# genglongling/EE274_ConvexCaldera_LLM_quantization

Hardware: AMD Instinct MI355X
Metric: weight matrices/sec (4096x4096, rank-128, Q=2-bit) + Frob err vs ref (higher is better)
Workload: dtype f32 (fp16 W in; fp32-grade split-fp16 MFMA products, fp64 small solves; int2 codes)

## Files before the change

ee274_convexcaldera_llm_quantization_amd/csrc/cq_small.hip:

```cpp
#include "cq_common.h"

namespace cq {

constexpr int GT = 64;
constexpr int GK = 32;
constexpr int kGramThreads = 256;

__global__ __launch_bounds__(kGramThreads) void gram_f64_kernel(
    int64_t M, int64_t N, int64_t K, int64_t kchunk, int splits, const float* __restrict__ A,
    int ta, int64_t lda, int64_t sa, const float* __restrict__ B, int tb, int64_t ldb, int64_t sb,
    double* __restrict__ part, const int* __restrict__ active) {
    __shared__ float As[GK][GT + 1];
    __shared__ float Bs[GK][GT + 1];
    const int64_t b = blockIdx.z / splits;
    if (active && !active[b]) return;
    const int split = blockIdx.z % splits;
    const int64_t i0 = (int64_t)blockIdx.y * GT, j0 = (int64_t)blockIdx.x * GT;
    const float* Ab = A + b * sa;
    const float* Bb = B + b * sb;
    const int tx = threadIdx.x & 15, ty = threadIdx.x >> 4;
    double acc[4][4];
#pragma unroll
    for (int u = 0; u < 4; ++u)
#pragma unroll
        for (int v = 0; v < 4; ++v) acc[u][v] = 0.0;
    const int64_t kbeg = split * kchunk, kend = min(K, kbeg + kchunk);
    for (int64_t k0 = kbeg; k0 < kend; k0 += GK) {
        for (int e = threadIdx.x; e < GK * GT; e += kGramThreads) {
            int kk, ii;
            if (!ta) { kk = e / GT; ii = e % GT; } else { ii = e / GK; kk = e % GK; }
            const int64_t gk = k0 + kk, gi = i0 + ii;
            float v = 0.f;
            if (gk < kend && gi < M) v = ta ? Ab[gi * lda + gk] : Ab[gk * lda + gi];
            As[kk][ii] = v;
            int jj;
            if (!tb) { kk = e / GT; jj = e % GT; } else { jj = e / GK; kk = e % GK; }
            const int64_t gk2 = k0 + kk, gj = j0 + jj;
            float w = 0.f;
            if (gk2 < kend && gj < N) w = tb ? Bb[gj * ldb + gk2] : Bb[gk2 * ldb + gj];
            Bs[kk][jj] = w;
        }
        __syncthreads();
#pragma unroll 4
        for (int kk = 0; kk < GK; ++kk) {
            double av[4], bv[4];
#pragma unroll
            for (int u = 0; u < 4; ++u) av[u] = (double)As[kk][ty * 4 + u];
#pragma unroll
            for (int v = 0; v < 4; ++v) bv[v] = (double)Bs[kk][tx * 4 + v];
#pragma unroll
            for (int u = 0; u < 4; ++u)
#pragma unroll
                for (int v = 0; v < 4; ++v) acc[u][v] = fma(av[u], bv[v], acc[u][v]);
        }
        __syncthreads();
    }
    double* P = part + ((int64_t)b * splits + split) * M * N;
#pragma unroll
    for (int u = 0; u < 4; ++u)
#pragma unroll
        for (int v = 0; v < 4; ++v) {
            const int64_t i = i0 + ty * 4 + u, j = j0 + tx * 4 + v;
            if (i < M && j < N) P[i * N + j] = acc[u][v];
        }
}

__global__ void gram_reduce_kernel(const double* __restrict__ part, int64_t MN, int splits,
                                   int64_t batch, double* __restrict__ C, const int* __restrict__ active) {
    const int64_t total = batch * MN;
    for (int64_t e = (int64_t)blockIdx.x * blockDim.x + threadIdx.x; e < total;
         e += (int64_t)gridDim.x * blockDim.x) {
        const int64_t b = e / MN, o = e % MN;
        if (active && !active[b]) continue;
        double s = 0.0;
        for (int t = 0; t < splits; ++t) s += part[(b * splits + t) * MN + o];
        C[e] = s;
    }
}


using f64x4v = __attribute__((ext_vector_type(4))) double;

template <bool TK>
__global__ __launch_bounds__(kGramThreads) void gram_f64_mfma_kernel(
    int64_t M, int64_t N, int64_t K, int64_t kchunk, int splits, const float* __restrict__ A,
    int64_t lda, int64_t sa, const float* __restrict__ B, int64_t ldb, int64_t sb, int sym,
    double* __restrict__ part, double* __restrict__ C, const int* __restrict__ active) {
    constexpr int GP = TK ? GT + 4 : GT + 16;
    __shared__ float As[2][GK][GP];
    __shared__ float Bs[2][GK][GP];
    const int64_t b = blockIdx.z / splits;
    const int split = blockIdx.z % splits;
    if (sym && blockIdx.x < blockIdx.y) return;
    if (active && !active[b]) return;
    const int64_t i0 = (int64_t)blockIdx.y * GT, j0 = (int64_t)blockIdx.x * GT;
    const float* Ab = A + b * sa;
    const float* Bb = B + b * sb;
    const int t = threadIdx.x, lane = t & 63, wid = t >> 6;
    const int wi = wid >> 1, wj = wid & 1;
    const int lr = t >> 4, lc = (t & 15) * 4;
    const int tr = t >> 3, tk = (t & 7) * 4;
    const int64_t kbeg = split * kchunk, kend = min(K, kbeg + kchunk);
    auto ld4 = [&](const float* base, int64_t ld, int64_t lim, int64_t k, int64_t c0) -> float4 {
        float4 v = make_float4(0.f, 0.f, 0.f, 0.f);
        if (k < kend) {
            const float* src = base + k * ld + c0;
            if (c0 + 3 < lim) v = *reinterpret_cast<const float4*>(src);
            else {
                if (c0 < lim) v.x = src[0];
                if (c0 + 1 < lim) v.y = src[1];
                if (c0 + 2 < lim) v.z = src[2];
            }
        }
        return v;
    };
    f64x4v acc[2][2];
#pragma unroll
    for (int u = 0; u < 2; ++u)
#pragma unroll
        for (int v = 0; v < 2; ++v) acc[u][v] = f64x4v{0.0, 0.0, 0.0, 0.0};
    float4 ra[2], rb[2];
    auto ld4t = [&](const float* base, int64_t ld, int64_t lim, int64_t row, int64_t k) -> float4 {
        float4 v = make_float4(0.f, 0.f, 0.f, 0.f);
        if (row < lim && k < kend) {
            const float* src = base + row * ld + k;
            if (k + 3 < kend) v = *reinterpret_cast<const float4*>(src);
            else {
                v.x = src[0];
                if (k + 1 < kend) v.y = src[1];
                if (k + 2 < kend) v.z = src[2];
            }
        }
        return v;
    };
    auto fetch = [&](int64_t k0) {
#pragma unroll
        for (int h = 0; h < 2; ++h) {
            if constexpr (TK) {
                ra[h] = ld4t(Ab, lda, M, i0 + tr + 32 * h, k0 + tk);
                rb[h] = ld4t(Bb, ldb, N, j0 + tr + 32 * h, k0 + tk);
            } else {
                ra[h] = ld4(Ab, lda, M, k0 + lr + 16 * h, i0 + lc);
                rb[h] = ld4(Bb, ldb, N, k0 + lr + 16 * h, j0 + lc);
            }
        }
    };
    auto stash = [&](int buf) {
#pragma unroll
        for (int h = 0; h < 2; ++h) {
            if constexpr (TK) {
                const int c = tr + 32 * h;
                As[buf][tk + 0][c] = ra[h].x; As[buf][tk + 1][c] = ra[h].y;
                As[buf][tk + 2][c] = ra[h].z; As[buf][tk + 3][c] = ra[h].w;
                Bs[buf][tk + 0][c] = rb[h].x; Bs[buf][tk + 1][c] = rb[h].y;
                Bs[buf][tk + 2][c] = rb[h].z; Bs[buf][tk + 3][c] = rb[h].w;
            } else {
                *reinterpret_cast<float4*>(&As[buf][lr + 16 * h][lc]) = ra[h];
                *reinterpret_cast<float4*>(&Bs[buf][lr + 16 * h][lc]) = rb[h];
            }
        }
    };
    const int nsl = (int)ceil_div(kend - kbeg, GK);
    if (nsl > 0) { fetch(kbeg); stash(0); }
    __syncthreads();
    const int li = lane & 15, lk = lane >> 4;
    for (int sl = 0; sl < nsl; ++sl) {
        const int cur = sl & 1;
        if (sl + 1 < nsl) fetch(kbeg + (int64_t)(sl + 1) * GK);
#pragma unroll
        for (int kk = 0; kk < GK; kk += 4) {
            double a0 = (double)As[cur][kk + lk][32 * wi + li];
            double a1 = (double)As[cur][kk + lk][32 * wi + 16 + li];
            double b0 = (double)Bs[cur][kk + lk][32 * wj + li];
            double b1 = (double)Bs[cur][kk + lk][32 * wj + 16 + li];
            acc[0][0] = __builtin_amdgcn_mfma_f64_16x16x4f64(a0, b0, acc[0][0], 0, 0, 0);
            acc[0][1] = __builtin_amdgcn_mfma_f64_16x16x4f64(a0, b1, acc[0][1], 0, 0, 0);
            acc[1][0] = __builtin_amdgcn_mfma_f64_16x16x4f64(a1, b0, acc[1][0], 0, 0, 0);
            acc[1][1] = __builtin_amdgcn_mfma_f64_16x16x4f64(a1, b1, acc[1][1], 0, 0, 0);
        }
        if (sl + 1 < nsl) stash(1 - cur);
        __syncthreads();
    }
    double* P = C ? C + (int64_t)b * M * N : part + ((int64_t)b * splits + split) * M * N;
    const bool mirror = C && sym && blockIdx.x != blockIdx.y;
#pragma unroll
    for (int u = 0; u < 2; ++u)
#pragma unroll
        for (int v = 0; v < 2; ++v)
#pragma unroll
            for (int r = 0; r < 4; ++r) {
                const int64_t i = i0 + 32 * wi + 16 * u + lk + 4 * r;
                const int64_t j = j0 + 32 * wj + 16 * v + li;
                if (i < M && j < N) {
                    const double x = C ? 0.0 + acc[u][v][r] : acc[u][v][r];
                    P[i * N + j] = x;
                    if (mirror) P[j * N + i] = x;
                }
            }
}

__global__ void gram_reduce_sym_kernel(const double* __restrict__ part, int64_t M, int splits,
                                       int64_t batch, double* __restrict__ C, const int* __restrict__ active) {
    const int64_t MN = M * M, total = batch * MN;
    for (int64_t e = (int64_t)blockIdx.x * blockDim.x + threadIdx.x; e < total;
         e += (int64_t)gridDim.x * blockDim.x) {
        const int64_t b = e / MN, o = e % MN, i = o / M, j = o % M;
        if (active && !active[b]) continue;
        const int64_t src = (i / GT > j / GT) ? j * M + i : o;
        double s = 0.0;
        for (int t2 = 0; t2 < splits; ++t2) s += part[(b * splits + t2) * MN + src];
        C[e] = s;
    }
}

static int gram_splits(int64_t M, int64_t N, int64_t K, int64_t batch) {
    const int64_t tiles = ceil_div(M, GT) * ceil_div(N, GT) * batch;
    int64_t s = ceil_div(1024, tiles);
    s = std::min<int64_t>(s, std::max<int64_t>(1, K / 256));
    return (int)std::max<int64_t>(1, std::min<int64_t>(s, 64));
}

template <int PPT, int RPT, int JBR, int NTH>
__global__ __launch_bounds__(NTH) void jacobi_reg_kernel(const double* __restrict__ A_all,
                                                                    int p, int max_sweeps, double tol,
                                                                    double* __restrict__ evals,
                                                                    float* __restrict__ V32,
                                                                    double* __restrict__ V64,
                                                                    int* __restrict__ sweeps_out,
                                                                    const int* __restrict__ active) {
    extern __shared__ __attribute__((aligned(16))) char smem_raw[];
    if (active && !active[blockIdx.x]) {
        if (threadIdx.x == 0 && sweeps_out) sweeps_out[blockIdx.x] = 0;
        return;
    }
    const int P = p + (p & 1);
    const int H = P / 2;
    double2* csn = reinterpret_cast<double2*>(smem_raw);
    int4* lohi = reinterpret_cast<int4*>(csn + H);
    int* flp = reinterpret_cast<int*>(lohi + H);
    int* seat = flp + H;
    int* seat2 = seat + P;
    int* rnk = seat2 + P;
    double* a = reinterpret_cast<double*>(rnk + P + ((9 * H + 3 * P) & 1));
    __shared__ double red[16];
    __shared__ int stop;
    const int64_t b = blockIdx.x;
    const double* Ag = A_all + b * (int64_t)p * p;
    const int tid = threadIdx.x, lane = tid & 63, wid = tid >> 6;
    const bool wantv = V32 != nullptr || V64 != nullptr;
    const int pg = lane & 31;
    const int rg = 2 * wid + (lane >> 5);
    const int k0 = pg * PPT, x0 = rg * RPT;
    auto pk = [p](int i, int j) -> int {
        if (i > j) { const int t = i; i = j; j = t; }
        return i * p - ((i * (i - 1)) >> 1) + (j - i);
    };
    auto pko = [p](int i) -> int { return i * p - ((i * (i - 1)) >> 1) - i; };
    auto pkx = [](int x, int ox, int y, int oy) -> int { return x <= y ? ox + y : oy + x; };
    for (int i = wid; i < p; i += (NTH / 64))
        for (int c = lane; c < p; c += 64)
            if (c >= i) a[pk(i, c)] = 0.5 * (Ag[i * p + c] + Ag[c * p + i]);
    for (int s = tid; s < P; s += NTH) seat[s] = s;
    float ev[PPT][RPT], od[PPT][RPT];
#pragma unroll
    for (int u = 0; u < PPT; ++u)
#pragma unroll
        for (int r = 0; r < RPT; ++r) {
            const int k = k0 + u, x = x0 + r;
            ev[u][r] = (x == 2 * k) ? 1.f : 0.f;
            od[u][r] = (x == 2 * k + 1) ? 1.f : 0.f;
        }
    __syncthreads();
    const double skip_rel = fmax(1e-17, 0.01 * tol);
    const double skip_rel2 = skip_rel * skip_rel;
    constexpr int JMB = 5;
    const int nblk = H * (H + 1) / 2;
    int bqa[JMB], bqb[JMB];
#pragma unroll
    for (int u = 0; u < JMB; ++u) {
        const int e = tid + u * NTH;
        bqa[u] = -1;
        bqb[u] = 0;
        if (JBR == 1 && e < nblk) {
            int qb = (int)((sqrtf(8.0f * (float)e + 1.0f) - 1.0f) * 0.5f);
            if (qb * (qb + 1) / 2 > e) --qb;
            if ((qb + 1) * (qb + 2) / 2 <= e) ++qb;
            bqa[u] = e - qb * (qb + 1) / 2;
            bqb[u] = qb;
        }
    }
    int* scur = seat;
    int* snxt = seat2;
    int sweep = 0;
    for (; sweep < max_sweeps; ++sweep) {
        double off = 0.0, dg = 0.0;
        for (int i = wid; i < p; i += (NTH / 64))
            for (int c = i + lane; c < p; c += 64) {
                const double v = a[pk(i, c)];
                if (c == i) dg += v * v; else off += 2.0 * v * v;
            }
        const double offs = block_sum_f64(off, red);
        const double dgs = block_sum_f64(dg, red);
        if (tid == 0) stop = (offs <= tol * tol * dgs) ? 1 : 0;
        __syncthreads();
        if (stop) break;
        for (int rd = 0; rd < P - 1; ++rd) {
            int act = 0;
            for (int k = tid; k < H; k += NTH) {
                const int se = scur[2 * k], so = scur[2 * k + 1];
                const int i = min(se, so), j = max(se, so);
                double c = 1.0, s = 0.0;
                if (j < p) {
                    const double aij = a[pk(i, j)];
                    const double aii = a[pk(i, i)], ajj = a[pk(j, j)];
                    if (fabs(aij) > 1e-300 && aij * aij > skip_rel2 * fabs(aii * ajj)) {
                        const double th = (ajj - aii) / (2.0 * aij);
                        const double t = (th >= 0 ? 1.0 : -1.0) / (fabs(th) + sqrt(1.0 + th * th));
                        c = 1.0 / sqrt(1.0 + t * t);
                        s = t * c;
                        act = 1;
                    }
                }
                csn[k] = make_double2(c, s); lohi[k] = make_int4(i, j, pko(i), pko(j)); flp[k] = se > so;
                snxt[2 * k] = (k == 0) ? se : (k == 1) ? scur[1] : scur[2 * k - 2];
                snxt[2 * k + 1] = (k == H - 1) ? se : scur[2 * k + 3];
            }
            const bool any = __syncthreads_or(act);
            if (any) {
                if constexpr (JBR == 1) {
#pragma unroll
                    for (int u = 0; u < JMB; ++u) {
                        const int qa = bqa[u], qb = bqb[u];
                        if (qa < 0) continue;
                        const double2 rca = csn[qa], rcb = csn[qb];
                        const double sa = rca.y, sb = rcb.y;
                        if (sa == 0.0 && sb == 0.0) continue;
                        const double ca = rca.x, cb = rcb.x;
                        const int4 pa = lohi[qa], pb = lohi[qb];
                        const int ia = pa.x, ja = pa.y, ib = pb.x, jb = pb.y;
                        const int oia = pa.z, oja = pa.w, oib = pb.z, ojb = pb.w;
                        const bool va = ja < p, vb = jb < p;
                        if (qa == qb) {
                            if (!va) continue;
                            const int o0 = pkx(ia, oia, ia, oia), o1 = pkx(ia, oia, ja, oja), o3 = pkx(ja, oja, ja, oja);
                            const double x0 = a[o0], x1 = a[o1], x3 = a[o3];
                            const double y00 = cb * x0 - sb * x1, y01 = sb * x0 + cb * x1;
                            const double y10 = cb * x1 - sb * x3, y11 = sb * x1 + cb * x3;
                            a[o0] = ca * y00 - sa * y10;
                            a[o3] = sa * y01 + ca * y11;
                            a[o1] = 0.0;
                        } else {
                            const int o0 = pkx(ia, oia, ib, oib);
                            const int o1 = vb ? pkx(ia, oia, jb, ojb) : -1;
                            const int o2 = va ? pkx(ja, oja, ib, oib) : -1;
                            const int o3 = (va && vb) ? pkx(ja, oja, jb, ojb) : -1;
                            const double x0 = a[o0];
                            const double x1 = o1 >= 0 ? a[o1] : 0.0;
                            const double x2 = o2 >= 0 ? a[o2] : 0.0;
                            const double x3 = o3 >= 0 ? a[o3] : 0.0;
                            const double y00 = cb * x0 - sb * x1, y01 = sb * x0 + cb * x1;
                            const double y10 = cb * x2 - sb * x3, y11 = sb * x2 + cb * x3;
                            a[o0] = ca * y00 - sa * y10;
                            if (o1 >= 0) a[o1] = ca * y01 - sa * y11;
                            if (o2 >= 0) a[o2] = sa * y00 + ca * y10;
                            if (o3 >= 0) a[o3] = sa * y01 + ca * y11;
                        }
                    }
                } else
                for (int e0 = tid; e0 < nblk; e0 += NTH * JBR) {
                    int o[JBR][4];
                    double x[JBR][4], ca[JBR], sa[JBR], cb[JBR], sb[JBR];
                    bool live[JBR], dgn[JBR];
#pragma unroll
                    for (int u = 0; u < JBR; ++u) {
                        const int e = e0 + u * NTH;
                        live[u] = false;
                        dgn[u] = false;
                        if (e < nblk) {
                            int qb = (int)((sqrtf(8.0f * (float)e + 1.0f) - 1.0f) * 0.5f);
                            if (qb * (qb + 1) / 2 > e) --qb;
                            if ((qb + 1) * (qb + 2) / 2 <= e) ++qb;
                            const int qa = e - qb * (qb + 1) / 2;
                            ca[u] = csn[qa].x; sa[u] = csn[qa].y; cb[u] = csn[qb].x; sb[u] = csn[qb].y;
                            const int ia = lohi[qa].x, ja = lohi[qa].y, ib = lohi[qb].x, jb = lohi[qb].y;
                            const bool va = ja < p, vb = jb < p;
                            if ((sa[u] != 0.0 || sb[u] != 0.0) && (qa != qb || va)) {
                                live[u] = true;
                                dgn[u] = (qa == qb);
                                if (dgn[u]) {
                                    o[u][0] = pk(ia, ia); o[u][1] = pk(ia, ja);
                                    o[u][2] = o[u][1]; o[u][3] = pk(ja, ja);
                                } else {
                                    o[u][0] = pk(ia, ib);
                                    o[u][1] = vb ? pk(ia, jb) : -1;
                                    o[u][2] = va ? pk(ja, ib) : -1;
                                    o[u][3] = (va && vb) ? pk(ja, jb) : -1;
                                }
#pragma unroll
                                for (int w4 = 0; w4 < 4; ++w4) x[u][w4] = o[u][w4] >= 0 ? a[o[u][w4]] : 0.0;
                            }
                        }
                    }
#pragma unroll
                    for (int u = 0; u < JBR; ++u) {
                        if (!live[u]) continue;
                        const double y00 = cb[u] * x[u][0] - sb[u] * x[u][1], y01 = sb[u] * x[u][0] + cb[u] * x[u][1];
                        const double y10 = cb[u] * x[u][2] - sb[u] * x[u][3], y11 = sb[u] * x[u][2] + cb[u] * x[u][3];
                        if (dgn[u]) {
                            a[o[u][0]] = ca[u] * y00 - sa[u] * y10;
                            a[o[u][3]] = sa[u] * y01 + ca[u] * y11;
                            a[o[u][1]] = 0.0;
                        } else {
                            a[o[u][0]] = ca[u] * y00 - sa[u] * y10;
                            if (o[u][1] >= 0) a[o[u][1]] = ca[u] * y01 - sa[u] * y11;
                            if (o[u][2] >= 0) a[o[u][2]] = sa[u] * y00 + ca[u] * y10;
                            if (o[u][3] >= 0) a[o[u][3]] = sa[u] * y01 + ca[u] * y11;
                        }
                    }
                }
#pragma unroll
                for (int u = 0; u < PPT; ++u) {
                    if (!wantv) break;
                    const int k = k0 + u;
                    if (k < H) {
                        const float c = (float)csn[k].x, s = (float)csn[k].y;
                        if (s != 0.f) {
                            const bool f = flp[k] != 0;
#pragma unroll
                            for (int r = 0; r < RPT; ++r) {
                                const float e = ev[u][r], o2 = od[u][r];
                                if (!f) { ev[u][r] = c * e - s * o2; od[u][r] = s * e + c * o2; }
                                else { od[u][r] = c * o2 - s * e; ev[u][r] = s * o2 + c * e; }
                            }
                        }
                    }
                }
            }
#pragma unroll
            for (int r = 0; r < RPT; ++r) {
                if (!wantv) break;
                const float from_left = __shfl_up(ev[PPT - 1][r], 1, 32);
                const float from_right = __shfl_down(od[0][r], 1, 32);
                float ne[PPT], no[PPT];
#pragma unroll
                for (int u = 0; u < PPT; ++u) {
                    const int k = k0 + u;
                    const float evm1 = (u == 0) ? from_left : ev[u - 1][r];
                    const float odp1 = (u == PPT - 1) ? from_right : od[u + 1][r];
                    ne[u] = (k == 0) ? ev[u][r] : (k == 1) ? od[u - (u > 0 ? 1 : 0)][r] : evm1;
                    no[u] = (k == H - 1) ? ev[u][r] : odp1;
                    if (k >= H) { ne[u] = ev[u][r]; no[u] = od[u][r]; }
                }
                const float od0_left = __shfl_up(od[PPT - 1][r], 1, 32);
                if (PPT == 1 && k0 == 1) ne[0] = od0_left;
#pragma unroll
                for (int u = 0; u < PPT; ++u) { ev[u][r] = ne[u]; od[u][r] = no[u]; }
            }
            __syncthreads();
            int* const t2 = scur;
            scur = snxt;
            snxt = t2;
        }
    }
    if (tid == 0 && sweeps_out) sweeps_out[b] = sweep;
    for (int i = tid; i < p; i += NTH) {
        const double di = a[pk(i, i)];
        int rank = 0;
        for (int j = 0; j < p; ++j) {
            const double dj = a[pk(j, j)];
            rank += (dj > di) || (dj == di && j < i);
        }
        evals[b * p + rank] = di;
        rnk[i] = rank;
    }
    __syncthreads();
#pragma unroll
    for (int u = 0; u < PPT; ++u) {
        const int k = k0 + u;
        if (k >= H) continue;
        const int pe = scur[2 * k], po = scur[2 * k + 1];
#pragma unroll
        for (int r = 0; r < RPT; ++r) {
            const int x = x0 + r;
            if (x >= p) continue;
            if (pe < p) {
                if (V32) V32[b * (int64_t)p * p + x * p + rnk[pe]] = ev[u][r];
                if (V64) V64[b * (int64_t)p * p + x * p + rnk[pe]] = ev[u][r];
            }
            if (po < p) {
                if (V32) V32[b * (int64_t)p * p + x * p + rnk[po]] = od[u][r];
                if (V64) V64[b * (int64_t)p * p + x * p + rnk[po]] = od[u][r];
            }
        }
    }
}

static size_t jacobi_reg_bytes(int p) {
    const int P = p + (p & 1), H = P / 2;
    return (size_t)2 * H * sizeof(double) + (size_t)(5 * H + 3 * P + 1) * sizeof(int) + 8 +
           (size_t)p * (p + 1) / 2 * sizeof(double) + 16;
}

constexpr int kWmThreads = 512;
__host__ __device__ inline int wm_pitch(int p) { return p + (48 - p % 32) % 32; }
constexpr int kWmWaves = kWmThreads / 64;


template <bool LP>
__global__ __launch_bounds__(kWmThreads) void spd_whiten_mfma_kernel(double* __restrict__ S_all, int p, double rc2,
                                                                     double* __restrict__ E_all,
                                                                     float* __restrict__ W32, int* __restrict__ info,
                                                                     const int* __restrict__ active) {
    extern __shared__ __attribute__((aligned(16))) double wm_smem[];
    if (active && !active[blockIdx.x]) return;
    double* piv = wm_smem;
    double* Li = piv + p;
    double* rp = Li + 32 * 33;
    double* Bk = rp + 32;
    const int pp = wm_pitch(p);
    double* PP = Bk + 32 * 33;
    __shared__ int bad;
    __shared__ double dmax_s;
    __shared__ double red[16];
    const int64_t b = blockIdx.x;
    double* S = S_all + b * (int64_t)p * p;
    double* E = E_all + b * (int64_t)p * p;
    const int tid = threadIdx.x, lane = tid & 63, wid = tid >> 6;
    const int l16 = lane & 15, lk = lane >> 4;
    for (int i = wid; i < p; i += kWmWaves)
        for (int c = lane; c < p; c += 64) E[(int64_t)i * p + c] = (i == c) ? 1.0 : 0.0;
    double dm = 0.0;
    for (int j = tid; j < p; j += kWmThreads) dm = fmax(dm, fabs(S[(int64_t)j * p + j]));
    for (int o = 32; o > 0; o >>= 1) {
        const int2 x = __builtin_bit_cast(int2, dm);
        int2 y;
        y.x = __shfl_xor(x.x, o, 64);
        y.y = __shfl_xor(x.y, o, 64);
        dm = fmax(dm, __builtin_bit_cast(double, y));
    }
    if (lane == 0) red[wid] = dm;
    if (tid == 0) bad = 0;
    __syncthreads();
    if (tid == 0) {
        double m = 0.0;
        for (int w = 0; w < kWmWaves; ++w) m = fmax(m, red[w]);
        dmax_s = m;
    }
    __syncthreads();
    const double dmax = dmax_s;
    for (int J = 0; J < p; J += 32) {
        const int nb = min(32, p - J);
        const int t0 = J + nb;
        {
            const int r = tid >> 4, c0 = tid & 15;
#pragma unroll
            for (int h = 0; h < 2; ++h) {
                const int c = c0 + 16 * h;
                const int a = min(r, c), e = max(r, c);
                Bk[r * 33 + c] = (r < nb && c < nb) ? S[(int64_t)(J + a) * p + J + e] : 0.0;
                Li[r * 33 + c] = (c == r) ? 1.0 : 0.0;
            }
            __syncthreads();
            int nbad = 0;
            for (int k = 0; k < nb; ++k) {
                const double d = Bk[k * 33 + k];
                const bool drop = !(d > 1e-300 && d > dmax * rc2);
                nbad += drop;
                if (tid == 0) {
                    piv[J + k] = drop ? __longlong_as_double(0x7ff0000000000000ll) : d;
                    rp[k] = drop ? 0.0 : 1.0 / d;
                }
                if (!drop && r > k && r < nb) {
                    const double f = Bk[r * 33 + k] / d;
#pragma unroll
                    for (int h = 0; h < 2; ++h) {
                        const int c = c0 + 16 * h;
                        if (c > k && c < nb) Bk[r * 33 + c] -= f * Bk[k * 33 + c];
                        else if (c <= k) Li[r * 33 + c] -= f * Li[k * 33 + c];
                    }
                }
                __syncthreads();
            }
            if (tid == 0) bad += nbad;
        }
        __syncthreads();
        const int ncs = (p - t0 + 15) / 16, nce = (t0 + 15) / 16;
        for (int cb = wid; cb < ncs + nce; cb += kWmWaves) {
            const bool isS = cb < ncs;
            double* M = isS ? S : E;
            const int c0 = isS ? t0 + 16 * cb : 16 * (cb - ncs);
            const int clim = isS ? p : t0;
            const int col = c0 + l16;
            f64x4v acc[2] = {f64x4v{0.0, 0.0, 0.0, 0.0}, f64x4v{0.0, 0.0, 0.0, 0.0}};
#pragma unroll
            for (int k0 = 0; k0 < 32; k0 += 4) {
                const int k = k0 + lk;
                const double bv = (k < nb && col < clim) ? M[(int64_t)(J + k) * p + col] : 0.0;
                acc[0] = __builtin_amdgcn_mfma_f64_16x16x4f64(Li[l16 * 33 + k], bv, acc[0], 0, 0, 0);
                acc[1] = __builtin_amdgcn_mfma_f64_16x16x4f64(Li[(16 + l16) * 33 + k], bv, acc[1], 0, 0, 0);
            }
#pragma unroll
            for (int h = 0; h < 2; ++h)
#pragma unroll
                for (int r = 0; r < 4; ++r) {
                    const int k = 16 * h + lk + 4 * r;
                    if (col < clim) {
                        const double v = k < nb ? acc[h][r] : 0.0;
                        if (LP) PP[k * pp + col] = v;
                        if ((!isS || !LP) && k < nb) M[(int64_t)(J + k) * p + col] = v;
                    }
                }
        }
        __syncthreads();
        const int nt = (p - t0 + 15) / 16;
        const int nst = nt * (nt + 1) / 2, net = nt * nce;
        auto tile_of = [&](int t, int& i0, int& c0, double*& M) {
            if (t < nst) {
                int tj = (int)((sqrtf(8.0f * (float)t + 1.0f) - 1.0f) * 0.5f);
                if (tj * (tj + 1) / 2 > t) --tj;
                if ((tj + 1) * (tj + 2) / 2 <= t) ++tj;
                i0 = t0 + 16 * (t - tj * (tj + 1) / 2);
                c0 = t0 + 16 * tj;
                M = S;
            } else {
                i0 = t0 + 16 * ((t - nst) / nce);
                c0 = 16 * ((t - nst) % nce);
                M = E;
            }
        };
        for (int t = wid; t < nst + net; t += 2 * kWmWaves) {
            const int tb = t + kWmWaves;
            const bool two = tb < nst + net;
            int i0[2] = {0, 0}, c0[2] = {0, 0};
            double* M[2] = {S, S};
            tile_of(t, i0[0], c0[0], M[0]);
            if (two) tile_of(tb, i0[1], c0[1], M[1]);
            double dv[2][4];
#pragma unroll
            for (int u = 0; u < 2; ++u) {
                const int clim = (M[u] == S) ? p : t0;
                const int col = c0[u] + l16;
#pragma unroll
                for (int r = 0; r < 4; ++r) {
                    const int i = i0[u] + lk + 4 * r;
                    dv[u][r] = (u == 0 || two) && i < p && col < clim ? M[u][(int64_t)i * p + col] : 0.0;
                }
            }
#pragma unroll
            for (int u = 0; u < 2; ++u) {
                if (u == 1 && !two) break;
                const int clim = (M[u] == S) ? p : t0;
                const int col = c0[u] + l16, arow = i0[u] + l16;
                f64x4v acc = f64x4v{0.0, 0.0, 0.0, 0.0};
#pragma unroll
                for (int k0 = 0; k0 < 32; k0 += 4) {
                    const int k = k0 + lk;
                    const bool kv = k < nb;
                    const double av = (kv && arow < p) ? (LP ? PP[k * pp + arow] : S[(int64_t)(J + k) * p + arow]) * rp[k] : 0.0;
                    const double bv = (kv && col < clim) ? (LP ? PP[k * pp + col] : M[u][(int64_t)(J + k) * p + col]) : 0.0;
                    acc = __builtin_amdgcn_mfma_f64_16x16x4f64(av, bv, acc, 0, 0, 0);
                }
#pragma unroll
                for (int r = 0; r < 4; ++r) {
                    const int i = i0[u] + lk + 4 * r;
                    if (i < p && col < clim) M[u][(int64_t)i * p + col] = dv[u][r] - acc[r];
                }
            }
        }
        __syncthreads();
    }
    if (tid == 0) info[b] = bad;
    for (int a = wid; a < p; a += kWmWaves)
        for (int c = lane; c < p; c += 64) {
            const double v = (c >= a) ? E[(int64_t)c * p + a] / sqrt(piv[c]) : 0.0;
            if (W32) W32[b * (int64_t)p * p + (int64_t)a * p + c] = (float)v;
            S[(int64_t)a * p + c] = v;
        }
}

constexpr int kLzThreads = 256, kLzMaxP = 192, kLzMaxPG = 512, kLzMaxSteps = 64;

__device__ __forceinline__ int lz_sturm(const double* al, const double* b2, int m, double x) {
    int cnt = 0;
    double d = 1.0;
    for (int k = 0; k < m; ++k) {
        d = (al[k] - x) - (k > 0 ? b2[k] / d : 0.0);
        if (d == 0.0) d = -1e-300;
        cnt += d < 0.0;
    }
    return cnt;
}

template <int Q, bool GT, int NT>
__global__ __launch_bounds__(NT) void extreme_eigs_kernel(const double* __restrict__ T_all, int p, int steps,
                                                         double* __restrict__ ends,
                                                         const int* __restrict__ active) {
    if (active && !active[blockIdx.x]) return;
    extern __shared__ __attribute__((aligned(16))) float lz_t[];
    __shared__ float vf[64 * Q];
    __shared__ float part[NT / 64][64 * Q];
    __shared__ double al[kLzMaxSteps], b2[kLzMaxSteps];
    __shared__ int m_s;
    const int64_t b = blockIdx.x;
    const double* T = T_all + b * (int64_t)p * p;
    const int tid = threadIdx.x, lane = tid & 63, wid = tid >> 6;
    if constexpr (!GT) {
        for (int e = tid; e < p * p; e += NT) lz_t[e] = (float)T[e];
        __syncthreads();
        for (int e = tid; e < p * p; e += NT) {
            const int j = e / p, i = e % p;
            if (i < j) {
                const float v = 0.5f * (lz_t[e] + lz_t[i * p + j]);
                lz_t[e] = v;
                lz_t[i * p + j] = v;
            }
        }
    }
    double v[Q], vp[Q];
#pragma unroll
    for (int q = 0; q < Q; ++q) v[q] = vp[q] = 0.0;
    if (wid == 0) {
        double ss = 0.0;
#pragma unroll
        for (int q = 0; q < Q; ++q) {
            const int i = lane + 64 * q;
            if (i < p) {
                uint32_t h = (uint32_t)i * 2654435761u ^ 0x9E3779B9u;
                h ^= h >> 16; h *= 0x7feb352du; h ^= h >> 15;
                v[q] = ((double)(h & 0xffffu) / 65536.0 + 0.5) * ((h & 0x10000u) ? 1.0 : -1.0);
                ss += v[q] * v[q];
            }
        }
        const double inv = 1.0 / sqrt(wave_sum(ss));
#pragma unroll
        for (int q = 0; q < Q; ++q) {
            v[q] *= inv;
            if (lane + 64 * q < p) vf[lane + 64 * q] = (float)v[q];
        }
        if (lane == 0) m_s = steps;
    }
    __syncthreads();
    constexpr int NWV = NT / 64;
    const int jc = (p + NWV - 1) / NWV, j0 = wid * jc, j1 = min(p, j0 + jc);
    double beta = 0.0;
    for (int k = 0; k < steps; ++k) {
        {
            int ii[Q];
            float a[Q];
#pragma unroll
            for (int q = 0; q < Q; ++q) {
                ii[q] = lane + 64 * q < p ? lane + 64 * q : 0;
                a[q] = 0.f;
            }
            int j = j0;
            for (; j + 4 <= j1; j += 4) {
                float t[4][Q], vj[4];
#pragma unroll
                for (int u = 0; u < 4; ++u) {
                    vj[u] = vf[j + u];
#pragma unroll
                    for (int q = 0; q < Q; ++q)
                        t[u][q] = GT ? (float)T[(int64_t)(j + u) * p + ii[q]] : lz_t[(j + u) * p + ii[q]];
                }
#pragma unroll
                for (int u = 0; u < 4; ++u)
#pragma unroll
                    for (int q = 0; q < Q; ++q) a[q] = __builtin_fmaf(t[u][q], vj[u], a[q]);
            }
            for (; j < j1; ++j) {
                const float vj = vf[j];
#pragma unroll
                for (int q = 0; q < Q; ++q)
                    a[q] = __builtin_fmaf(GT ? (float)T[(int64_t)j * p + ii[q]] : lz_t[j * p + ii[q]], vj, a[q]);
            }
#pragma unroll
            for (int q = 0; q < Q; ++q)
                if (lane + 64 * q < p) part[wid][lane + 64 * q] = a[q];
        }
        __syncthreads();
        if (wid == 0) {
            double w[Q], a = 0.0;
#pragma unroll
            for (int q = 0; q < Q; ++q) {
                const int i = lane + 64 * q;
                w[q] = 0.0;
                if (i < p) {
                    double acc = 0.0;
#pragma unroll
                    for (int wv = 0; wv < NWV; ++wv) acc += (double)part[wv][i];
                    w[q] = acc;
                    w[q] -= beta * vp[q];
                    a += w[q] * v[q];
                }
            }
            a = wave_sum(a);
            double ss = 0.0;
#pragma unroll
            for (int q = 0; q < Q; ++q) {
                w[q] -= a * v[q];
                ss += w[q] * w[q];
            }
            ss = wave_sum(ss);
            if (lane == 0) {
                al[k] = a;
                b2[k + 1 < kLzMaxSteps ? k + 1 : 0] = ss;
            }
            beta = sqrt(ss);
            const int stop = !(beta > 1e-30 * fabs(a)) || k + 1 == steps;
            if (stop && lane == 0) m_s = k + 1;
            const double inv = stop ? 0.0 : 1.0 / beta;
#pragma unroll
            for (int q = 0; q < Q; ++q) {
                vp[q] = v[q];
                v[q] = w[q] * inv;
                if (lane + 64 * q < p) vf[lane + 64 * q] = (float)v[q];
            }
        }
        __syncthreads();
        if (m_s != steps || k + 1 == steps) break;
    }
    const int m = m_s;
    if (wid < 2) {
        double lo = INFINITY, hi = -INFINITY;
        for (int k = 0; k < m; ++k) {
            const double r = (k > 0 ? sqrt(b2[k]) : 0.0) + (k + 1 < m ? sqrt(b2[k + 1]) : 0.0);
            lo = fmin(lo, al[k] - r);
            hi = fmax(hi, al[k] + r);
        }
        const double pad = 1e-12 * fmax(fabs(lo), fabs(hi)) + 1e-300;
        double a = lo - pad, c = hi + pad;
        bool bad = !(a == a) || !(c == c);
        for (int it = 0; it < 9 && !bad; ++it) {
            const double x = a + (c - a) * (double)(lane + 1) / 65.0;
            const int cnt = lz_sturm(al, b2, m, x);
            if (wid == 0) {
                const uint64_t msk = __ballot(cnt == m);
                const int jf = msk ? __builtin_ctzll(msk) : 64;
                const double nc = jf < 64 ? a + (c - a) * (double)(jf + 1) / 65.0 : c;
                const double na = jf > 0 ? a + (c - a) * (double)jf / 65.0 : a;
                a = na; c = nc;
            } else {
                const uint64_t msk = __ballot(cnt == 0);
                const int jl = __builtin_popcountll(msk);
                const double na = jl > 0 ? a + (c - a) * (double)jl / 65.0 : a;
                const double nc = jl < 64 ? a + (c - a) * (double)(jl + 1) / 65.0 : c;
                a = na; c = nc;
            }
        }
        if (lane == 0) ends[2 * b + wid] = bad ? NAN : 0.5 * (a + c);
    }
}

__global__ __launch_bounds__(256) void ritz_partial_kernel(const float* __restrict__ X,
                                                            const float* __restrict__ Z,
                                                            const double* __restrict__ theta,
                                                            int64_t k, int64_t p, int64_t r,
                                                            int64_t rows_per, double* part,
                                                            const int* __restrict__ active) {
    const int64_t b = blockIdx.y, chunk = blockIdx.x;
    if (active && !active[b]) return;
    const int64_t r0 = chunk * rows_per, r1 = min(k, r0 + rows_per);
    for (int64_t c = threadIdx.x; c < r; c += blockDim.x) {
        const float th = (float)theta[b * p + c];
        double s = 0.0;
        for (int64_t i = r0; i < r1; ++i) {
            const float d = Z[b * k * p + i * p + c] - th * X[b * k * p + i * p + c];
            s += (double)d * d;
        }
        part[(b * gridDim.x + chunk) * r + c] = s;
    }
}

__global__ void ritz_final_kernel(const double* part, int nchunks, int64_t p, int64_t r,
                                  const double* theta, float* out, const int* __restrict__ active) {
    __shared__ double red[16];
    const int64_t b = blockIdx.x;
    if (active && !active[b]) return;
    double mx = 0.0;
    for (int64_t c = threadIdx.x; c < r; c += blockDim.x) {
        double s = 0.0;
        for (int t = 0; t < nchunks; ++t) s += part[(b * nchunks + t) * r + c];
        mx = fmax(mx, sqrt(s));
    }
    for (int off = 32; off > 0; off >>= 1) mx = fmax(mx, __shfl_xor(mx, off, 64));
    if ((threadIdx.x & 63) == 0) red[threadIdx.x >> 6] = mx;
    __syncthreads();
    if (threadIdx.x == 0) {
        double m = 0.0;
        for (int i = 0; i < (int)(blockDim.x >> 6); ++i) m = fmax(m, red[i]);
        const double t0 = fabs(theta[b * p]);
        out[b] = (float)(t0 > 0 ? m / t0 : m);
    }
}

__global__ void ritz_prod_final_kernel(const double* part, int nchunks, int64_t p, int64_t r,
                                       const double* theta, const double* ysq, float* out,
                                       const int* __restrict__ active) {
    __shared__ double red[16];
    const int64_t b = blockIdx.x;
    if (active && !active[b]) return;
    const double t0 = fabs(theta[b * p]), tp = theta[b * p + p - 1];
    double acc = 0.0;
    for (int64_t c = threadIdx.x; c < r; c += blockDim.x) {
        double s = 0.0;
        for (int t = 0; t < nchunks; ++t) s += part[(b * nchunks + t) * r + c];
        const double th = fmax(theta[b * p + c], 0.0);
        const double gap = fmax(th - tp, 1e-3 * t0);
        acc += s * th / (gap * gap);
    }
    acc = wave_sum(acc);
    if ((threadIdx.x & 63) == 0) red[threadIdx.x >> 6] = acc;
    __syncthreads();
    if (threadIdx.x == 0) {
        double a = 0.0;
        for (int i = 0; i < (int)(blockDim.x >> 6); ++i) a += red[i];
        const double y2 = ysq[b];
        out[b] = (float)(y2 > 0 ? sqrt(a / y2) : sqrt(a));
    }
}

}

using namespace cq;

extern "C" {

size_t cq_gram_f64_workspace(int64_t M, int64_t N, int64_t K, int64_t batch) {
    return (size_t)batch * gram_splits(M, N, K, batch) * M * N * sizeof(double);
}

int cq_gram_f64(int64_t M, int64_t N, int64_t K, int64_t batch, const float* A, int trans_a,
                int64_t lda, int64_t stride_a, const float* B, int trans_b, int64_t ldb,
                int64_t stride_b, double* C, void* ws, size_t ws_bytes, void* stream) {
    return cq_gram_f64_masked(M, N, K, batch, A, trans_a, lda, stride_a, B, trans_b, ldb, stride_b, C, nullptr, ws,
                              ws_bytes, stream);
}

int cq_gram_f64_masked(int64_t M, int64_t N, int64_t K, int64_t batch, const float* A, int trans_a,
                       int64_t lda, int64_t stride_a, const float* B, int trans_b, int64_t ldb,
                       int64_t stride_b, double* C, const int* active, void* ws, size_t ws_bytes, void* stream) {
    CQ_REQUIRE(A && B && C && M > 0 && N > 0 && K > 0 && batch > 0, "cq_gram_f64: bad args");
    const int splits = gram_splits(M, N, K, batch);
    if (!ws || ws_bytes < cq_gram_f64_workspace(M, N, K, batch))
        return set_error(CQ_EWORKSPACE, "cq_gram_f64: workspace too small");
    CQ_REQUIRE(batch * splits <= 65535, "cq_gram_f64: batch too large");
    const int64_t kchunk = ceil_div(ceil_div(K, splits), GK) * GK;
    hipStream_t s = as_stream(stream);
    dim3 grid((unsigned)ceil_div(N, GT), (unsigned)ceil_div(M, GT), (unsigned)(batch * splits));
    const int64_t tot = batch * M * N;
    const unsigned rgrid = (unsigned)std::min<int64_t>(ceil_div(tot, 256), 4096);
    const bool al4 = lda % 4 == 0 && ldb % 4 == 0 && stride_a % 4 == 0 && stride_b % 4 == 0 &&
                     reinterpret_cast<uintptr_t>(A) % 16 == 0 && reinterpret_cast<uintptr_t>(B) % 16 == 0;
    if (al4 && trans_a == trans_b) {
        const int sym = (A == B && lda == ldb && stride_a == stride_b && M == N) ? 1 : 0;
        double* direct = splits == 1 ? C : nullptr;
        if (trans_a)
            gram_f64_mfma_kernel<true><<<grid, kGramThreads, 0, s>>>(M, N, K, kchunk, splits, A, lda, stride_a, B,
                                                                     ldb, stride_b, sym, reinterpret_cast<double*>(ws),
                                                                     direct, active);
        else
            gram_f64_mfma_kernel<false><<<grid, kGramThreads, 0, s>>>(M, N, K, kchunk, splits, A, lda, stride_a, B,
                                                                      ldb, stride_b, sym, reinterpret_cast<double*>(ws),
                                                                      direct, active);
        if (direct) return check_launch("cq_gram_f64");
        if (sym)
            gram_reduce_sym_kernel<<<rgrid, 256, 0, s>>>(reinterpret_cast<double*>(ws), M, splits, batch, C, active);
        else
            gram_reduce_kernel<<<rgrid, 256, 0, s>>>(reinterpret_cast<double*>(ws), M * N, splits, batch, C, active);
        return check_launch("cq_gram_f64");
    }
    gram_f64_kernel<<<grid, kGramThreads, 0, s>>>(M, N, K, kchunk, splits, A, trans_a, lda,
                                                   stride_a, B, trans_b, ldb, stride_b,
                                                   reinterpret_cast<double*>(ws), active);
    gram_reduce_kernel<<<rgrid, 256, 0, s>>>(reinterpret_cast<double*>(ws), M * N, splits, batch, C, active);
    return check_launch("cq_gram_f64");
}

int cq_spd_whiten(double* S, int64_t p, int64_t batch, float* Wt32, double* Wt64, int* info,
                  void* stream) {
    return cq_spd_whiten_rcond(S, p, batch, 1e-30, Wt32, Wt64, info, stream);
}

int cq_spd_whiten_rcond(double* S, int64_t p, int64_t batch, double rcond2, float* Wt32, double* Wt64, int* info,
                        void* stream) {
    return cq_spd_whiten_masked(S, p, batch, rcond2, Wt32, Wt64, info, nullptr, stream);
}

int cq_spd_whiten_masked(double* S, int64_t p, int64_t batch, double rcond2, float* Wt32, double* Wt64, int* info,
                         const int* active, void* stream) {
    CQ_REQUIRE(S && p > 0 && batch > 0 && info && Wt64, "cq_spd_whiten: bad args (Wt64 is required scratch)");
    CQ_REQUIRE(rcond2 >= 0.0, "cq_spd_whiten: rcond2 must be >= 0");
    hipStream_t s = as_stream(stream);
    const size_t wsm = (size_t)(p + 2 * 32 * 33 + 32) * sizeof(double);
    const size_t wlm = wsm + (size_t)32 * wm_pitch((int)p) * sizeof(double);
    CQ_REQUIRE(wsm <= 64 * 1024, "cq_spd_whiten: p too large");
    if (wlm <= 150 * 1024)
        spd_whiten_mfma_kernel<true><<<(unsigned)batch, kWmThreads, wlm, s>>>(S, (int)p, rcond2, Wt64, Wt32, info, active);
    else
        spd_whiten_mfma_kernel<false><<<(unsigned)batch, kWmThreads, wsm, s>>>(S, (int)p, rcond2, Wt64, Wt32, info, active);
    return check_launch("cq_spd_whiten");
}

size_t cq_jacobi_workspace(int64_t p, int64_t batch) {
    if (p > kBlockJacobiMinP) return cq::bj_workspace(p, batch);
    return 16;
}

int cq_jacobi_eigh(double* A, int64_t p, int64_t batch, int max_sweeps, double tol, double* evals,
                   float* V32, double* V64, int* sweeps_out, void* ws, size_t ws_bytes,
                   void* stream) {
    return cq_jacobi_eigh_masked(A, p, batch, max_sweeps, tol, evals, V32, V64, sweeps_out, nullptr, ws, ws_bytes,
                                 stream);
}

int cq_jacobi_eigh_masked(double* A, int64_t p, int64_t batch, int max_sweeps, double tol, double* evals,
                          float* V32, double* V64, int* sweeps_out, const int* active, void* ws, size_t ws_bytes,
                          void* stream) {
    CQ_REQUIRE(A && evals && p > 0 && batch > 0 && max_sweeps > 0, "cq_jacobi_eigh: bad args");
    CQ_REQUIRE(p <= 4096, "cq_jacobi_eigh: p too large");
    if (!ws || ws_bytes < cq_jacobi_workspace(p, batch))
        return set_error(CQ_EWORKSPACE, "cq_jacobi_eigh: workspace too small");
    hipStream_t s = as_stream(stream);
    if (p > kBlockJacobiMinP)
        return cq::bj_eigh(A, p, batch, max_sweeps, tol, evals, V32, V64, sweeps_out, active, ws, ws_bytes, s);
    const size_t lreg = jacobi_reg_bytes((int)p);
    CQ_REQUIRE(lreg <= 160 * 1024, "cq_jacobi_eigh: LDS budget");
    if (p <= 64)
        jacobi_reg_kernel<1, 2, 2, 1024><<<(unsigned)batch, 1024, lreg, s>>>(A, (int)p, max_sweeps, tol, evals, V32, V64, sweeps_out, active);
    else if (p <= 128)
        jacobi_reg_kernel<2, 4, 2, 1024><<<(unsigned)batch, 1024, lreg, s>>>(A, (int)p, max_sweeps, tol, evals, V32, V64, sweeps_out, active);
    else
        jacobi_reg_kernel<3, 6, 1, 1024><<<(unsigned)batch, 1024, lreg, s>>>(A, (int)p, max_sweeps, tol, evals, V32, V64, sweeps_out, active);
    return check_launch("cq_jacobi_eigh");
}

size_t cq_jacobi_staged_workspace(int64_t p, int64_t batch) { return cq::bj_workspace(p, batch); }

int cq_jacobi_eigh_staged(double* A, int64_t p, int64_t batch, int phase, int nsweeps, double tol, int want_vectors,
                          double* evals, float* V32, double* V64, int* sweeps_out, int* pending_out, void* ws,
                          size_t ws_bytes, void* stream) {
    return cq_jacobi_eigh_staged_masked(A, p, batch, phase, nsweeps, tol, want_vectors, evals, V32, V64, sweeps_out,
                                        pending_out, nullptr, ws, ws_bytes, stream);
}

int cq_jacobi_eigh_staged_masked(double* A, int64_t p, int64_t batch, int phase, int nsweeps, double tol,
                                 int want_vectors, double* evals, float* V32, double* V64, int* sweeps_out,
                                 int* pending_out, const int* active, void* ws, size_t ws_bytes, void* stream) {
    CQ_REQUIRE(A && p >= 2 && p <= 4096 && batch > 0, "cq_jacobi_eigh_staged: bad args");
    CQ_REQUIRE(phase > 0 && phase <= (BJ_BEGIN | BJ_SWEEPS | BJ_END), "cq_jacobi_eigh_staged: bad phase");
    CQ_REQUIRE(!(phase & BJ_SWEEPS) || nsweeps > 0, "cq_jacobi_eigh_staged: nsweeps must be > 0");
    CQ_REQUIRE(!(phase & BJ_END) || (evals && (!want_vectors || V32 || V64)), "cq_jacobi_eigh_staged: outputs");
    if (!ws || ws_bytes < cq_jacobi_staged_workspace(p, batch))
        return set_error(CQ_EWORKSPACE, "cq_jacobi_eigh_staged: workspace too small");
    return cq::bj_stage(A, p, batch, phase, nsweeps, tol, want_vectors != 0, evals, V32, V64, sweeps_out, pending_out,
                        active, ws, ws_bytes, as_stream(stream));
}

int cq_extreme_eigs(const double* T, int64_t p, int64_t batch, int steps, double* ends, void* stream) {
    return cq_extreme_eigs_masked(T, p, batch, steps, ends, nullptr, stream);
}

int cq_extreme_eigs_masked(const double* T, int64_t p, int64_t batch, int steps, double* ends, const int* active,
                           void* stream) {
    CQ_REQUIRE(T && ends && p >= 2 && batch > 0 && batch <= 2147483647, "cq_extreme_eigs: bad args");
    CQ_REQUIRE(p <= kLzMaxPG, "cq_extreme_eigs: p > %d", kLzMaxPG);
    CQ_REQUIRE(steps >= 1 && steps < kLzMaxSteps, "cq_extreme_eigs: steps must be in [1, %d)", kLzMaxSteps);
    hipStream_t s = as_stream(stream);
    if (p <= kLzMaxP)
        extreme_eigs_kernel<3, false, kLzThreads><<<(unsigned)batch, kLzThreads, (size_t)p * p * sizeof(float), s>>>(
            T, (int)p, steps, ends, active);
    else if (p <= 320)
        extreme_eigs_kernel<5, true, 1024><<<(unsigned)batch, 1024, 0, s>>>(T, (int)p, steps, ends, active);
    else if (p <= 384)
        extreme_eigs_kernel<6, true, 1024><<<(unsigned)batch, 1024, 0, s>>>(T, (int)p, steps, ends, active);
    else
        extreme_eigs_kernel<8, true, 1024><<<(unsigned)batch, 1024, 0, s>>>(T, (int)p, steps, ends, active);
    return check_launch("cq_extreme_eigs");
}

size_t cq_ritz_workspace(int64_t k, int64_t r, int64_t batch) {
    const int64_t nch = std::min<int64_t>(64, std::max<int64_t>(1, k / 64));
    return (size_t)batch * nch * r * sizeof(double);
}

int cq_ritz_residual(const float* X, const float* Z, const double* theta, int64_t k, int64_t p,
                     int64_t r, int64_t batch, float* out, void* ws, size_t ws_bytes,
                     void* stream) {
    return cq_ritz_residual_masked(X, Z, theta, k, p, r, batch, out, nullptr, ws, ws_bytes, stream);
}

int cq_ritz_residual_masked(const float* X, const float* Z, const double* theta, int64_t k, int64_t p,
                            int64_t r, int64_t batch, float* out, const int* active, void* ws, size_t ws_bytes,
                            void* stream) {
    CQ_REQUIRE(X && Z && theta && out && k > 0 && p > 0 && r > 0 && r <= p, "cq_ritz_residual: bad args");
    if (!ws || ws_bytes < cq_ritz_workspace(k, r, batch))
        return set_error(CQ_EWORKSPACE, "cq_ritz_residual: workspace too small");
    hipStream_t s = as_stream(stream);
    const int64_t nch = std::min<int64_t>(64, std::max<int64_t>(1, k / 64));
    const int64_t rows_per = ceil_div(k, nch);
    double* part = reinterpret_cast<double*>(ws);
    ritz_partial_kernel<<<dim3((unsigned)nch, (unsigned)batch), 256, 0, s>>>(X, Z, theta, k, p, r, rows_per, part, active);
    ritz_final_kernel<<<(unsigned)batch, 256, 0, s>>>(part, (int)nch, p, r, theta, out, active);
    return check_launch("cq_ritz_residual");
}

int cq_ritz_product_error(const float* X, const float* Z, const double* theta, int64_t k, int64_t p, int64_t r,
                          int64_t batch, const double* ysq, float* out, void* ws, size_t ws_bytes, void* stream) {
    return cq_ritz_product_error_masked(X, Z, theta, k, p, r, batch, ysq, out, nullptr, ws, ws_bytes, stream);
}

int cq_ritz_product_error_masked(const float* X, const float* Z, const double* theta, int64_t k, int64_t p, int64_t r,
                                 int64_t batch, const double* ysq, float* out, const int* active, void* ws,
                                 size_t ws_bytes, void* stream) {
    CQ_REQUIRE(X && Z && theta && ysq && out && k > 0 && p > 0 && r > 0 && r < p,
               "cq_ritz_product_error: bad args");
    if (!ws || ws_bytes < cq_ritz_workspace(k, r, batch))
        return set_error(CQ_EWORKSPACE, "cq_ritz_product_error: workspace too small");
    hipStream_t s = as_stream(stream);
    const int64_t nch = std::min<int64_t>(64, std::max<int64_t>(1, k / 64));
    const int64_t rows_per = ceil_div(k, nch);
    double* part = reinterpret_cast<double*>(ws);
    ritz_partial_kernel<<<dim3((unsigned)nch, (unsigned)batch), 256, 0, s>>>(X, Z, theta, k, p, r, rows_per, part, active);
    ritz_prod_final_kernel<<<(unsigned)batch, 256, 0, s>>>(part, (int)nch, p, r, theta, ysq, out, active);
    return check_launch("cq_ritz_product_error");
}

}
```

Measured before the change: 355.9.

## Deepen gram MFMA prefetch to a three-slot register ring with specialized paths

Replaces the single register prefetch in the f64 MFMA gram kernel with a ring of three register sets, so global loads are issued several K-slices ahead of the MFMA work that consumes them. Interior tiles get a specialization with no bounds checks. Diagonal tiles of symmetric grams skip loading and storing B and read A's shared tile instead. It also adds a launch-bounds occupancy hint of 3 blocks per CU. The cost is more registers per thread and four template instantiations, which may limit occupancy or grow code size.

```diff
diff --git a/ee274_convexcaldera_llm_quantization_amd/csrc/cq_small.hip b/ee274_convexcaldera_llm_quantization_amd/csrc/cq_small.hip
--- a/ee274_convexcaldera_llm_quantization_amd/csrc/cq_small.hip
+++ b/ee274_convexcaldera_llm_quantization_amd/csrc/cq_small.hip
@@ -80,9 +80,12 @@
 
 
 using f64x4v = __attribute__((ext_vector_type(4))) double;
+using f32x4v = __attribute__((ext_vector_type(4))) float;
+constexpr int GR = 3;
+template <int N> using gr_c = std::integral_constant<int, N>;
 
 template <bool TK>
-__global__ __launch_bounds__(kGramThreads) void gram_f64_mfma_kernel(
+__global__ __launch_bounds__(kGramThreads, 3) void gram_f64_mfma_kernel(
     int64_t M, int64_t N, int64_t K, int64_t kchunk, int splits, const float* __restrict__ A,
     int64_t lda, int64_t sa, const float* __restrict__ B, int64_t ldb, int64_t sb, int sym,
     double* __restrict__ part, double* __restrict__ C, const int* __restrict__ active) {
@@ -101,11 +104,11 @@
     const int lr = t >> 4, lc = (t & 15) * 4;
     const int tr = t >> 3, tk = (t & 7) * 4;
     const int64_t kbeg = split * kchunk, kend = min(K, kbeg + kchunk);
-    auto ld4 = [&](const float* base, int64_t ld, int64_t lim, int64_t k, int64_t c0) -> float4 {
-        float4 v = make_float4(0.f, 0.f, 0.f, 0.f);
+    auto ld4 = [&](const float* base, int64_t ld, int64_t lim, int64_t k, int64_t c0) -> f32x4v {
+        f32x4v v = f32x4v{0.f, 0.f, 0.f, 0.f};
         if (k < kend) {
             const float* src = base + k * ld + c0;
-            if (c0 + 3 < lim) v = *reinterpret_cast<const float4*>(src);
+            if (c0 + 3 < lim) v = *reinterpret_cast<const f32x4v*>(src);
             else {
                 if (c0 < lim) v.x = src[0];
                 if (c0 + 1 < lim) v.y = src[1];
@@ -119,12 +122,11 @@
     for (int u = 0; u < 2; ++u)
 #pragma unroll
         for (int v = 0; v < 2; ++v) acc[u][v] = f64x4v{0.0, 0.0, 0.0, 0.0};
-    float4 ra[2], rb[2];
-    auto ld4t = [&](const float* base, int64_t ld, int64_t lim, int64_t row, int64_t k) -> float4 {
-        float4 v = make_float4(0.f, 0.f, 0.f, 0.f);
+    auto ld4t = [&](const float* base, int64_t ld, int64_t lim, int64_t row, int64_t k) -> f32x4v {
+        f32x4v v = f32x4v{0.f, 0.f, 0.f, 0.f};
         if (row < lim && k < kend) {
             const float* src = base + row * ld + k;
-            if (k + 3 < kend) v = *reinterpret_cast<const float4*>(src);
+            if (k + 3 < kend) v = *reinterpret_cast<const f32x4v*>(src);
             else {
                 v.x = src[0];
                 if (k + 1 < kend) v.y = src[1];
@@ -133,53 +135,120 @@
         }
         return v;
     };
-    auto fetch = [&](int64_t k0) {
-#pragma unroll
-        for (int h = 0; h < 2; ++h) {
-            if constexpr (TK) {
-                ra[h] = ld4t(Ab, lda, M, i0 + tr + 32 * h, k0 + tk);
-                rb[h] = ld4t(Bb, ldb, N, j0 + tr + 32 * h, k0 + tk);
-            } else {
-                ra[h] = ld4(Ab, lda, M, k0 + lr + 16 * h, i0 + lc);
-                rb[h] = ld4(Bb, ldb, N, k0 + lr + 16 * h, j0 + lc);
-            }
-        }
+    const int nsl = (int)ceil_div(kend - kbeg, GK);
+    const int li = lane & 15, lk = lane >> 4;
+    const bool interior = i0 + GT <= M && j0 + GT <= N && kend - kbeg == (int64_t)nsl * GK;
+    const bool diag = sym && blockIdx.x == blockIdx.y;
+    auto run = [&](auto in_c, auto dg_c) {
+        constexpr bool IN = decltype(in_c)::value, DG = decltype(dg_c)::value;
+        struct Set { f32x4v a[2], b[2]; };
+        Set r0, r1, r2;
+        static_assert(GR == 3, "the ring names GR register sets");
+        auto set = [&](auto s_c) -> Set& {
+            constexpr int S = decltype(s_c)::value % GR;
+            if constexpr (S == 0) return r0;
+            else if constexpr (S == 1) return r1;
+            else return r2;
+        };
+        int64_t kf = kbeg;
+        auto fetch = [&](Set& r) {
+#pragma unroll
+            for (int h = 0; h < 2; ++h) {
+                if constexpr (TK) {
+                    if constexpr (IN) {
+                        r.a[h] = *reinterpret_cast<const f32x4v*>(Ab + (i0 + tr + 32 * h) * lda + kf + tk);
+                        if constexpr (!DG)
+                            r.b[h] = *reinterpret_cast<const f32x4v*>(Bb + (j0 + tr + 32 * h) * ldb + kf + tk);
+                    } else {
+                        r.a[h] = ld4t(Ab, lda, M, i0 + tr + 32 * h, kf + tk);
+                        if constexpr (!DG) r.b[h] = ld4t(Bb, ldb, N, j0 + tr + 32 * h, kf + tk);
+                    }
+                } else {
+                    if constexpr (IN) {
+                        r.a[h] = *reinterpret_cast<const f32x4v*>(Ab + (kf + lr + 16 * h) * lda + i0 + lc);
+                        if constexpr (!DG)
+                            r.b[h] = *reinterpret_cast<const f32x4v*>(Bb + (kf + lr + 16 * h) * ldb + j0 + lc);
+                    } else {
+                        r.a[h] = ld4(Ab, lda, M, kf + lr + 16 * h, i0 + lc);
+                        if constexpr (!DG) r.b[h] = ld4(Bb, ldb, N, kf + lr + 16 * h, j0 + lc);
+                    }
+                }
+            }
+            kf += GK;
+        };
+        auto stash = [&](const Set& r, int buf) {
+#pragma unroll
+            for (int h = 0; h < 2; ++h) {
+                if constexpr (TK) {
+                    const int c = tr + 32 * h;
+                    As[buf][tk + 0][c] = r.a[h].x; As[buf][tk + 1][c] = r.a[h].y;
+                    As[buf][tk + 2][c] = r.a[h].z; As[buf][tk + 3][c] = r.a[h].w;
+                    if constexpr (!DG) {
+                        Bs[buf][tk + 0][c] = r.b[h].x; Bs[buf][tk + 1][c] = r.b[h].y;
+                        Bs[buf][tk + 2][c] = r.b[h].z; Bs[buf][tk + 3][c] = r.b[h].w;
+                    }
+                } else {
+                    *reinterpret_cast<f32x4v*>(&As[buf][lr + 16 * h][lc]) = r.a[h];
+                    if constexpr (!DG) *reinterpret_cast<f32x4v*>(&Bs[buf][lr + 16 * h][lc]) = r.b[h];
+                }
+            }
+        };
+        auto mult = [&](int cur) {
+            const float (*Bc)[GP] = DG ? As[cur] : Bs[cur];
+#pragma unroll
+            for (int kk = 0; kk < GK; kk += 4) {
+                double a0 = (double)As[cur][kk + lk][32 * wi + li];
+                double a1 = (double)As[cur][kk + lk][32 * wi + 16 + li];
+                double b0 = (double)Bc[kk + lk][32 * wj + li];
+                double b1 = (double)Bc[kk + lk][32 * wj + 16 + li];
+                acc[0][0] = __builtin_amdgcn_mfma_f64_16x16x4f64(a0, b0, acc[0][0], 0, 0, 0);
+                acc[0][1] = __builtin_amdgcn_mfma_f64_16x16x4f64(a0, b1, acc[0][1], 0, 0, 0);
+                acc[1][0] = __builtin_amdgcn_mfma_f64_16x16x4f64(a1, b0, acc[1][0], 0, 0, 0);
+                acc[1][1] = __builtin_amdgcn_mfma_f64_16x16x4f64(a1, b1, acc[1][1], 0, 0, 0);
+            }
+        };
+        fetch(r0);
+        if (nsl > 1) fetch(r1);
+        if (nsl > 2) fetch(r2);
+        stash(r0, 0);
+        __syncthreads();
+        int sl = 0;
+        auto step = [&](auto s_c) {
+            constexpr int S = decltype(s_c)::value;
+            const int cur = (sl + S) & 1;
+            fetch(set(s_c));
+            mult(cur);
+            stash(set(gr_c<S + 1>{}), 1 - cur);
+            __syncthreads();
+        };
+        for (; sl + 2 * GR <= nsl; sl += GR) {
+            step(gr_c<0>{});
+            step(gr_c<1>{});
+            step(gr_c<2>{});
+        }
+        auto last = [&](auto s_c) {
+            constexpr int S = decltype(s_c)::value;
+            if (sl + S >= nsl) return;
+            const int cur = (sl + S) & 1;
+            if (sl + S + GR < nsl) fetch(set(s_c));
+            mult(cur);
+            if (sl + S + 1 < nsl) stash(set(gr_c<S + 1>{}), 1 - cur);
+            __syncthreads();
+        };
+        last(gr_c<0>{});
+        last(gr_c<1>{});
+        last(gr_c<2>{});
+        last(gr_c<3>{});
+        last(gr_c<4>{});
     };
-    auto stash = [&](int buf) {
-#pragma unroll
-        for (int h = 0; h < 2; ++h) {
-            if constexpr (TK) {
-                const int c = tr + 32 * h;
-                As[buf][tk + 0][c] = ra[h].x; As[buf][tk + 1][c] = ra[h].y;
-                As[buf][tk + 2][c] = ra[h].z; As[buf][tk + 3][c] = ra[h].w;
-                Bs[buf][tk + 0][c] = rb[h].x; Bs[buf][tk + 1][c] = rb[h].y;
-                Bs[buf][tk + 2][c] = rb[h].z; Bs[buf][tk + 3][c] = rb[h].w;
-            } else {
-                *reinterpret_cast<float4*>(&As[buf][lr + 16 * h][lc]) = ra[h];
-                *reinterpret_cast<float4*>(&Bs[buf][lr + 16 * h][lc]) = rb[h];
-            }
-        }
-    };
-    const int nsl = (int)ceil_div(kend - kbeg, GK);
-    if (nsl > 0) { fetch(kbeg); stash(0); }
-    __syncthreads();
-    const int li = lane & 15, lk = lane >> 4;
-    for (int sl = 0; sl < nsl; ++sl) {
-        const int cur = sl & 1;
-        if (sl + 1 < nsl) fetch(kbeg + (int64_t)(sl + 1) * GK);
-#pragma unroll
-        for (int kk = 0; kk < GK; kk += 4) {
-            double a0 = (double)As[cur][kk + lk][32 * wi + li];
-            double a1 = (double)As[cur][kk + lk][32 * wi + 16 + li];
-            double b0 = (double)Bs[cur][kk + lk][32 * wj + li];
-            double b1 = (double)Bs[cur][kk + lk][32 * wj + 16 + li];
-            acc[0][0] = __builtin_amdgcn_mfma_f64_16x16x4f64(a0, b0, acc[0][0], 0, 0, 0);
-            acc[0][1] = __builtin_amdgcn_mfma_f64_16x16x4f64(a0, b1, acc[0][1], 0, 0, 0);
-            acc[1][0] = __builtin_amdgcn_mfma_f64_16x16x4f64(a1, b0, acc[1][0], 0, 0, 0);
-            acc[1][1] = __builtin_amdgcn_mfma_f64_16x16x4f64(a1, b1, acc[1][1], 0, 0, 0);
-        }
-        if (sl + 1 < nsl) stash(1 - cur);
-        __syncthreads();
+    if (nsl > 0) {
+        if (interior) {
+            if (diag) run(std::true_type{}, std::true_type{});
+            else run(std::true_type{}, std::false_type{});
+        } else {
+            if (diag) run(std::false_type{}, std::true_type{});
+            else run(std::false_type{}, std::false_type{});
+        }
     }
     double* P = C ? C + (int64_t)b * M * N : part + ((int64_t)b * splits + split) * M * N;
     const bool mirror = C && sym && blockIdx.x != blockIdx.y;
```

New measurement: 359.2, median of 6. No clear change (+0.9%).
